# lorenzsp/EMRI_FrequencyDomainWaveforms

Hardware: AMD Instinct MI355X
Metric: FD waveforms/sec (2 yr, dt=10 s, ~3000 modes) at 1/2/4/8 GPUs; mode-sum HBM GB/s (higher is better)
Workload: dtype f64

## Files before the change

emri_frequencydomainwaveforms_amd/csrc/emrifd.hip:

```cpp

#include <hip/hip_runtime.h>

#include <cmath>
#include <cstdint>
#include <cstdlib>
#include <cstdio>
#include <algorithm>
#include <atomic>
#include <mutex>
#include <cstring>
#include <string>
#include <type_traits>

#include "../../include/emrifd.h"

#define EFD_VERSION 100

namespace {

constexpr int TILE = 256;
constexpr int NWAVE = TILE / 64;
#ifndef EFD_BPL
#define EFD_BPL 3
#endif
// ... 1141 lines not shown
        const int src = __ffsll((long long)sel) - 1;
        lg.m = __shfl(m, src, 64);
        lg.n = __shfl(n, src, 64);
        const int kg = __shfl(key, src, 64);
        const bool mine = lane < K && key == kg;
        if (mine) s_mem[eqb] = lane;
        lg.count = __popcll(__ballot(mine));
    }
    __syncthreads();
    return lg;
}
__global__ __launch_bounds__(64) void k_prep_pcr_b(const PrepBatch B) {
    PREP_WALKER(B);
    if (!(D.pcr & 1) || (int)blockIdx.x >= 4 + ((D.pcr & 2) ? 5 : 1) * D.K) return;
    const GroupAmpSrc ga{D.amp, D.ylm_p, D.ylm_m, D.sc_re, D.sc_im,
                         ws_at<int32_t>(W, L.gstart), ws_at<int32_t>(W, L.gmem)};
    __shared__ int s_mem[PCR_GROUPS_MAX_K];
    LocalGroups lg{};
    if (B.pcr_groups && (blockIdx.x == 0 || blockIdx.x >= 4))
        lg = pcr_local_groups(D, W, L, s_mem);
    prep_pcr_body(D.t, D.phi_phi, D.phi_r, D.f_phi, D.f_r, ga, lg, ws_at<int32_t>(W, L.gm),
                  ws_at<int32_t>(W, L.gn), D.nt, D.K,
                  ws_at<double>(W, L.coefT), ws_at<double>(W, L.kslope), ws_at<double>(W, L.coefA),
                  ws_at<int32_t>(W, L.runs), ws_at<Item>(W, L.items), ws_at<double>(W, L.invcp),
                  ws_at<double>(W, L.invdp), ws_at<Header>(W, L.header));
}

__global__ __launch_bounds__(64) void k_spline_shared(const double* __restrict__ x, int n,
                                                      const double* __restrict__ y, int ninterp,
                                                      double* coef, int64_t scratch_stride) {
    auto yf = [&](int i, int q) { return y[(size_t)i * ninterp + q]; };
    spline_shared(x, n, yf, ninterp, ninterp, coef, scratch_stride, blockIdx.x);
}

template <bool UPPER>
__device__ int64_t grid_bound(const double* __restrict__ f, int64_t nf, double v, int64_t g) {
    auto pred = [&](int64_t i) { return UPPER ? (f[i] > v) : (f[i] >= v); };
    g = g < 0 ? 0 : (g > nf ? nf : g);
    int64_t lo, hi;
    if (g < nf && !pred(g)) {
        lo = g + 1;
        int64_t step = 1;
        while (true) {
            const int64_t p = lo + step - 1;
            if (p >= nf) { hi = nf; break; }
            if (pred(p)) { hi = p; break; }
            lo = p + 1;
            step <<= 1;
        }
    } else {
        hi = g;
        int64_t step = 1;
        while (true) {
            const int64_t p = hi - step;
            if (p < 0) { lo = 0; break; }
            if (pred(p)) { hi = p; step <<= 1; }
            else { lo = p + 1; break; }
        }
    }
    while (lo < hi) {
        const int64_t mid = (lo + hi) >> 1;
        if (pred(mid)) hi = mid; else lo = mid + 1;
    }
    return lo;
}

__device__ bool build_item(
    const double* __restrict__ t, const double* __restrict__ f_phi, const double* __restrict__ f_r,
    const int32_t* __restrict__ gm, const int32_t* __restrict__ gn, int ni, int K,
    const double* __restrict__ coefA, const double* __restrict__ coefT,
    const int32_t* __restrict__ runs, const double* __restrict__ freq, int64_t nf, int paired,
    int64_t nl, int64_t nl1, Item* __restrict__ items, int4* __restrict__ ranges, int h, int j,
    unsigned long long& evals, bool env);

__device__ __forceinline__ void items_body(const double* __restrict__ t, const double* __restrict__ f_phi,
                        const double* __restrict__ f_r, const int32_t* __restrict__ gm,
                        const int32_t* __restrict__ gn, const int32_t* __restrict__ gstart,
                        int nt, int K, const double* __restrict__ coefA,
                        const double* __restrict__ coefT, const int32_t* __restrict__ runs,
                        const double* __restrict__ freq, int64_t nf, int paired, int64_t nl,
                        int64_t nl1, Item* __restrict__ items, int4* __restrict__ ranges,
                        Header* __restrict__ hdr, bool runs_mark, bool env) {
    const int ni = nt - 1;
    const int G = hdr->groups;
    const int64_t total = (int64_t)ni * G;
    if ((int64_t)blockIdx.x * blockDim.x >= total) return;
    const int64_t stride = (int64_t)gridDim.x * blockDim.x;
    __shared__ unsigned long long red[3][4];
    unsigned long long ev = 0, contrib = 0, eev = 0;
    for (int64_t gid = (int64_t)blockIdx.x * blockDim.x + threadIdx.x; gid < total;
         gid += stride) {
        const int g = (int)(gid % G), j = (int)(gid / G);
        if (runs_mark && j == 0 && runs[(size_t)g * 4 * MAXRUNS + 3] != 0)
            atomicOr(&hdr->runs_overflow, 1);
        unsigned long long e1 = 0;
        const bool envr = build_item(t, f_phi, f_r, gm, gn, ni, K, coefA, coefT, runs, freq, nf,
                                     paired, nl, nl1, items, ranges, g, j, e1, env);
        ev += e1;
        contrib += e1 * (unsigned long long)(gstart[g + 1] - gstart[g]);
        eev += envr ? e1 : 0;
    }
    for (int o = 32; o > 0; o >>= 1) {
        ev += __shfl_xor(ev, o);
        contrib += __shfl_xor(contrib, o);
        eev += __shfl_xor(eev, o);
    }
    if ((threadIdx.x & 63) == 0) {
        red[0][threadIdx.x >> 6] = contrib;
        red[1][threadIdx.x >> 6] = ev;
        red[2][threadIdx.x >> 6] = eev;
    }
    __syncthreads();
    if (threadIdx.x == 0) {
        const unsigned long long c = red[0][0] + red[0][1] + red[0][2] + red[0][3];
        const unsigned long long e = red[1][0] + red[1][1] + red[1][2] + red[1][3];
        const unsigned long long x = red[2][0] + red[2][1] + red[2][2] + red[2][3];
        if (c) atomicAdd((unsigned long long*)&hdr->contributions, c);
        if (e) atomicAdd((unsigned long long*)&hdr->evaluations, e);
        if (x) atomicAdd((unsigned long long*)&hdr->env_evaluations, x);
    }
}
__global__ __launch_bounds__(256) void k_items(const PrepBatch B) {
    PREP_WALKER(B);
    items_body(D.t, D.f_phi, D.f_r, ws_at<int32_t>(W, L.gm), ws_at<int32_t>(W, L.gn),
               ws_at<int32_t>(W, L.gstart), D.nt, D.K, ws_at<double>(W, L.coefA),
               ws_at<double>(W, L.coefT), ws_at<int32_t>(W, L.runs), D.freq, B.nf, B.paired, B.nl,
               B.nl1, ws_at<Item>(W, L.items), ws_at<int4>(W, L.ranges),
               ws_at<Header>(W, L.header), (D.pcr & 1) != 0, D.env != 0);
}

template <class FAT>
__device__ bool record_safe(const Item& it, FAT fat, int64_t lo0, int64_t hi0, int64_t lo1,
                            int64_t hi1) {
    double ga = INFINITY, gb = -INFINITY;
    if (hi0 > lo0) {
        const double fa = fat(0, lo0), fb = fat(1, hi0 - 1);
        ga = fmin(ga, fmin(-fa, -fb));
        gb = fmax(gb, fmax(-fa, -fb));
    }
    if (hi1 > lo1) {
        const double fa = fat(2, lo1), fb = fat(3, hi1 - 1);
        ga = fmin(ga, fmin(fa, fb));
        gb = fmax(gb, fmax(fa, fb));
    }
    if (!(ga <= gb)) return false;
    auto wat = [&](double g) {
        const double u = g - it.gx;
        const double tt = fma(fma(fma(it.ic[0], u, it.ic[1]), u, it.ic[2]), u, it.ic[3]);
        return tt - it.tj;
    };
    const double wa = wat(ga), wb = wat(gb);
    const double mg = 1e-6 * it.dtj;
    if (!(fmin(wa, wb) >= mg && fmax(wa, wb) <= it.dtj - mg)) return false;
    const double ua = ga - it.gx, ub = gb - it.gx;
    auto dt = [&](double u) { return fma(fma(3.0 * it.ic[0], u, 2.0 * it.ic[1]), u, it.ic[2]); };
    const double da = dt(ua), db = dt(ub);
    if (!((da > 0.0 && db > 0.0) || (da < 0.0 && db < 0.0))) return false;
    if (it.ic[0] != 0.0) {
        const double uv = -it.ic[1] / (3.0 * it.ic[0]);
        if (uv > ua && uv < ub) {
            const double dv = dt(uv);
            if (!((dv > 0.0) == (da > 0.0) && dv != 0.0)) return false;
        }
    }
    const double* f = it.fd;
    const double scale = fabs(f[0]) * it.dtj * it.dtj + fabs(f[1]) * it.dtj + fabs(f[2]);
    const double sg = (it.fdneg & 1) ? -1.0 : 1.0;
    auto fq = [&](double x) { return sg * fma(fma(f[0], x, f[1]), x, f[2]); };
    double fmn = fmin(fq(0.0), fq(it.dtj));
    if (f[0] != 0.0) {
        const double xv = -f[1] / (2.0 * f[0]);
        if (xv > 0.0 && xv < it.dtj) fmn = fmin(fmn, fq(xv));
    }
    return fmn > 1e-12 * scale && isfinite(scale);
}

__device__ bool build_item(
    const double* __restrict__ t, const double* __restrict__ f_phi, const double* __restrict__ f_r,
    const int32_t* __restrict__ gm, const int32_t* __restrict__ gn, int ni, int K,
    const double* __restrict__ coefA, const double* __restrict__ coefT,
    const int32_t* __restrict__ runs, const double* __restrict__ freq, int64_t nf, int paired,
    int64_t nl, int64_t nl1, Item* __restrict__ items, int4* __restrict__ ranges, int h, int j,
    unsigned long long& evals, bool env) {
    Item& it = items[(size_t)h * ni + j];
    const int m = gm[h], n = gn[h];
    const int32_t* rr = runs + (size_t)h * 4 * MAXRUNS;
    int run = -1;
    for (int r = 0; r < MAXRUNS; ++r) {
        if (rr[4 * r + 2] != 0 && j >= rr[4 * r] && j < rr[4 * r + 1]) { run = r; break; }
    }
    const int partner = (m != 0) ? 1 : 0;
    evals = 0;
    it.fdneg = 0;
    if (run < 0) {
        it.klo[0] = it.khi[0] = it.klo[1] = it.khi[1] = 0;
        ranges[(size_t)h * ni + j] = make_int4(0, 0, 0, 0);
        return false;
    }
    const int a = rr[4 * run], sg = rr[4 * run + 2];
    it.tj = t[j];
    it.dtj = t[j + 1] - t[j];
    const double dm = (double)m, dn = (double)n;
    for (int c = 0; c < 4; ++c) {
        const double* ca = coefA + ((size_t)j * 4 + c) * 4 * K + 4 * h;
        it.b[0][0][c] = ca[0];
        it.b[0][1][c] = ca[1];
        it.b[1][0][c] = ca[2];
        it.b[1][1][c] = ca[3];
        const double* ct = coefT + ((size_t)j * 4 + c) * 8;
        it.ph[c] = dm * ct[0] + dn * ct[1];
    }
    double gq[3], ymin_rec;
    {
        const double* ct = coefT + (size_t)j * 32;
        const double F0 = dm * ct[0 * 8 + 2] + dn * ct[0 * 8 + 3];
        const double F1 = dm * ct[1 * 8 + 2] + dn * ct[1 * 8 + 3];
        const double F2 = dm * ct[2 * 8 + 2] + dn * ct[2 * 8 + 3];
        it.fd[0] = 3.0 * F0; it.fd[1] = 2.0 * F1; it.fd[2] = F2;
        const double G0 = dm * ct[0 * 8 + 4] + dn * ct[0 * 8 + 5];
        const double G1 = dm * ct[1 * 8 + 4] + dn * ct[1 * 8 + 5];
        const double G2 = dm * ct[2 * 8 + 4] + dn * ct[2 * 8 + 5];
        it.fdd[0] = FDD_SCALE * (3.0 * G0);
        it.fdd[1] = FDD_SCALE * (2.0 * G1);
        it.fdd[2] = FDD_SCALE * G2;
        const double dt = it.dtj;
        auto qv = [](double a, double b, double c, double x) { return (a * x + b) * x + c; };
        const double fa = it.fd[2], fb = qv(it.fd[0], it.fd[1], it.fd[2], dt);
        it.fdneg = qv(it.fd[0], it.fd[1], it.fd[2], 0.5 * dt) < 0.0 ? 1 : 0;
        double fdmin = fmin(fabs(fa), fabs(fb));
        if ((fa > 0.0) != (fb > 0.0) || fa == 0.0 || fb == 0.0) fdmin = 0.0;
        if (it.fd[0] != 0.0) {
            const double xv = -it.fd[1] / (2.0 * it.fd[0]);
            if (xv > 0.0 && xv < dt) {
                const double fv = qv(it.fd[0], it.fd[1], it.fd[2], xv);
                if ((fv > 0.0) != (fa > 0.0)) fdmin = 0.0;
                fdmin = fmin(fdmin, fabs(fv));
            }
        }
        double gmax = fmax(fabs(G2), fabs(qv(3.0 * G0, 2.0 * G1, G2, dt)));
        if (G0 != 0.0) {
            const double xv = -(2.0 * G1) / (6.0 * G0);
            if (xv > 0.0 && xv < dt) gmax = fmax(gmax, fabs(qv(3.0 * G0, 2.0 * G1, G2, xv)));
        }
        const double ymin = gmax > 0.0 ? TWO_PI * fdmin * fdmin * fdmin / (3.0 * gmax * gmax) / 1.1
                                       : INFINITY;
        int J = FAST_J;
        for (int jj = 1; jj < FAST_J; ++jj)
            if (ymin >= JSER_Y[jj]) { J = jj; break; }
        it.jser = J;
        gq[0] = 3.0 * G0; gq[1] = 2.0 * G1; gq[2] = G2;
        ymin_rec = ymin;
    }
    const double Fj = knotF(f_phi, f_r, m, n, j), Fj1 = knotF(f_phi, f_r, m, n, j + 1);
    const double xlo = sg > 0 ? Fj : Fj1;
    const double xhi = sg > 0 ? Fj1 : Fj;
    const bool strict_lo = sg > 0 ? (j == a) : (j + 1 == rr[4 * run + 1]);
    const double f0 = freq[0], span = freq[nf - 1] - f0;
    const double gsc = span > 0.0 ? (double)(nf - 1) / span : 0.0;
    auto guess = [&](double v) { return (int64_t)floor((v - f0) * gsc); };
    const double bv[4] = {-xhi, -xlo, xlo, xhi};
    const bool bu[4] = {true, !strict_lo, strict_lo, false};
    int64_t bg[4];
    double b3[4][3];
#pragma unroll
    for (int q = 0; q < 4; ++q) {
        const int64_t g = guess(bv[q]);
        bg[q] = g < 0 ? 0 : (g > nf ? nf : g);
    }
#pragma unroll
    for (int q = 0; q < 4; ++q) {
        const int64_t g = bg[q];
        b3[q][0] = freq[g >= 1 ? g - 1 : 0];
        b3[q][1] = freq[g < nf ? g : nf - 1];
        b3[q][2] = freq[g + 1 < nf ? g + 1 : nf - 1];
    }
    int64_t bk[4];
#pragma unroll
    for (int q = 0; q < 4; ++q) {
        const double v = bv[q];
        const int64_t g = bg[q];
        auto pred = [&](double x) { return bu[q] ? (x > v) : (x >= v); };
        int64_t k = -1;
        if (!(g >= 1 && pred(b3[q][0]))) {
            if (g == nf) k = nf;
            else if (pred(b3[q][1])) k = g;
            else if (g + 1 == nf) k = nf;
            else if (pred(b3[q][2])) k = g + 1;
        }
        if (k < 0)
            k = bu[q] ? grid_bound<true>(freq, nf, v, g) : grid_bound<false>(freq, nf, v, g);
        bk[q] = k;
    }
    int64_t lo0 = bk[0], hi0 = bk[1], lo1 = bk[2], hi1 = bk[3];
    const int64_t lim0 = paired ? nl : nf;
    const int64_t lim1 = paired ? nl1 : (partner ? nf : 0);
    auto clampr = [](int64_t& lo, int64_t& hi, int64_t lim) {
        if (lo > lim) lo = lim;
        if (hi > lim) hi = lim;
        if (hi < lo) hi = lo;
    };
    clampr(lo0, hi0, lim0);
    clampr(lo1, hi1, lim1);
    it.klo[0] = (int32_t)lo0; it.khi[0] = (int32_t)hi0;
    it.klo[1] = (int32_t)lo1; it.khi[1] = (int32_t)hi1;
    ranges[(size_t)h * ni + j] = make_int4((int)lo0, (int)hi0, (int)lo1, (int)hi1);
    auto fat = [&](int q, int64_t x) {
        const int64_t g = bg[q];
        if (g >= 1 && x == g - 1) return b3[q][0];
        if (g < nf && x == g) return b3[q][1];
        if (g + 1 < nf && x == g + 1) return b3[q][2];
        return freq[x];
    };
    if (record_safe(it, fat, lo0, hi0, lo1, hi1)) it.fdneg |= 2;
    const int mult = paired ? 1 + partner : 1;
    evals = (unsigned long long)((hi0 - lo0) + (hi1 - lo1)) * mult;
    if (env && (it.fdneg & 2) && ymin_rec >= ENV_MIN_Y && evals > 0) {
        EnvFit E;
        if (env_fit(it.fd, gq, it.dtj, (it.fdneg & 1) != 0, E)) {
            double* e = env_of(&it);
            for (int c = 0; c <= ENV_DEG; ++c) e[c] = E.a[c] * ENV_AMP_SCALE;
            for (int c = 0; c < 4; ++c) it.ph[c] -= E.th[c];
            it.jser = 0;
            return true;
        }
    }
    return false;
}

__device__ __forceinline__ void slot_segment(int i, const int32_t* __restrict__ runs,
                                             const int4* __restrict__ ranges, int nt, int G,
                                             int lim0, int lim1, int2& lh, int4& info) {
    const int h = i / (2 * MAXRUNS), r = (i >> 1) % MAXRUNS, sb = i & 1;
    const int ni = nt - 1;
    lh = make_int2(0, 0);
    info = make_int4(0, 0, 0, 0);
    const int32_t* rr = runs + (size_t)h * 4 * MAXRUNS + 4 * r;
    if (h < G && rr[2] != 0) {
        const int ja = rr[0], jb = rr[1], n = jb - ja;
        const int dir = (sb == 0) ? -rr[2] : rr[2];
        const int lim = sb ? lim1 : lim0;
        const int4* rg = ranges + (size_t)h * ni;
        int lo = 0, hi = n;
        while (lo < hi) {
            const int mid = (lo + hi) >> 1;
            const int4 v = rg[dir > 0 ? ja + mid : jb - 1 - mid];
            if ((sb ? v.w : v.y) > 0) hi = mid; else lo = mid + 1;
        }
        const int pa = lo;
        hi = n;
        while (lo < hi) {
            const int mid = (lo + hi) >> 1;
            const int4 v = rg[dir > 0 ? ja + mid : jb - 1 - mid];
            if ((sb ? v.z : v.x) >= lim) hi = mid; else lo = mid + 1;
        }
        const int pb = lo;
        if (pb > pa) {
            const int4 rf = rg[dir > 0 ? ja + pa : jb - 1 - pa];
            const int4 rl = rg[dir > 0 ? ja + pb - 1 : jb - pb];
            const int klo = sb ? rf.z : rf.x, khi = sb ? rl.w : rl.y;
            if (khi > klo) {
                lh = make_int2(klo, khi);
                const int jfirst = dir > 0 ? ja + pa : jb - pb;
                info = make_int4(h * ni + jfirst, pb - pa, dir, sb);
            }
        }
    }
}
__device__ __forceinline__ void segment_slots_body(const int32_t* __restrict__ runs,
                                                       const int4* __restrict__ ranges, int nt,
                                                       int K, int lim0, int lim1,
                                                       const Header* __restrict__ hdr,
                                                       int2* __restrict__ slot_lh,
                                                       int4* __restrict__ slot_info,
                                                       int32_t* __restrict__ blockcnt,
                                                       int32_t* __restrict__ blocktiles) {
    const int i = blockIdx.x * blockDim.x + threadIdx.x;
    __shared__ int wc[4], wt[4];
    int ntl = 0;
    bool valid = false;
    if (i < K * MAXRUNS * 2) {
        const int G = hdr->groups;
        int2 lh;
        int4 info;
        slot_segment(i, runs, ranges, nt, G, lim0, lim1, lh, info);
        slot_lh[i] = lh;
        slot_info[i] = info;
        valid = info.y > 0;
        if (valid) ntl = (lh.y - 1) / TILE_LANES - lh.x / TILE_LANES + 1;
    }
    const unsigned long long bal = __ballot(valid);
    int tsum = ntl;
    for (int o = 32; o > 0; o >>= 1) tsum += __shfl_xor(tsum, o);
    if ((threadIdx.x & 63) == 0) {
        wc[threadIdx.x >> 6] = __popcll(bal);
        wt[threadIdx.x >> 6] = tsum;
    }
    __syncthreads();
    if (threadIdx.x == 0) {
        blockcnt[blockIdx.x] = wc[0] + wc[1] + wc[2] + wc[3];
        blocktiles[blockIdx.x] = wt[0] + wt[1] + wt[2] + wt[3];
    }
}
__device__ __forceinline__ int slot_blocks(int K) { return (2 * MAXRUNS * K + 255) / 256; }
__global__ __launch_bounds__(256) void k_segment_slots(const PrepBatch B) {
    PREP_WALKER(B);
    if ((int)blockIdx.x >= slot_blocks(D.K)) return;
    segment_slots_body(ws_at<int32_t>(W, L.runs), ws_at<int4>(W, L.ranges), D.nt, D.K,
                       (int)(B.paired ? B.nl : B.nf), (int)(B.paired ? B.nl1 : B.nf),
                       ws_at<Header>(W, L.header), ws_at<int2>(W, L.slotlh),
// ... 1542 lines not shown
    const int32_t w_lo = (int32_t)(tile * TILE_LANES + wave * 64 * BPL);
    double llacc = 0.0;
#pragma unroll
    for (int i = 0; i < BPL; ++i) {
        const int64_t k = w_lo + 64 * i + lane;
        if (k >= nlanes) continue;
        const int64_t km = nf - 1 - k;
        double2 sk = make_double2(0.0, 0.0);
        double2 sm = make_double2(0.0, 0.0);
        if (km == k) {
            sk.x += sm.x;
            sk.y += sm.y;
            sm = sk;
        }
        auto put = [&](int64_t j, double2 a, double2 b) {
            if (j < k0) return;
            double2 vp = make_double2(0.5 * (a.x + b.x), 0.5 * (a.y - b.y));
            double2 vc = make_double2(-0.5 * (a.y + b.y), 0.5 * (a.x - b.x));
            {
#pragma clang fp contract(off)
                const int64_t q = j - k0, nb = nf - k0;
                const double2 d0 = reinterpret_cast<const double2*>(lld)[q];
                const double2 d1 = reinterpret_cast<const double2*>(lld)[nb + q];
                const double w0 = llw[q], w1 = llw[nb + q];
                const double r0 = d0.x - vp.x * w0, i0 = d0.y - vp.y * w0;
                const double r1 = d1.x - vc.x * w1, i1 = d1.y - vc.y * w1;
                llacc = fma(r0, r0, fma(i0, i0, llacc));
                llacc = fma(r1, r1, fma(i1, i1, llacc));
            }
        };
        put(km, sm, sk);
        if (km != k) put(k, sk, sm);
    }
#pragma unroll
    for (int o = 32; o > 0; o >>= 1) llacc += __shfl_xor(llacc, o, 64);
    __shared__ double llw4[NWAVE];
    if (lane == 0) llw4[wave] = llacc;
    __syncthreads();
    if (tid == 0) {
        double t = 0.0;
#pragma unroll
        for (int w = 0; w < NWAVE; ++w) t += llw4[w];
        llconst[tile] = t;
    }
}

struct LlBatch {
    const double* part[EFD_BATCH_MAX];
    const Header* hdr[EFD_BATCH_MAX];
    double* out;
    const double* llconst;
    int64_t ntiles;
    int32_t n;
};
struct StatusBatch {
    Header* h[EFD_BATCH_MAX];
    int32_t n;
};
__global__ __launch_bounds__(64) void k_lane_gather(const StatusBatch sb, int32_t* out) {
    const int i = threadIdx.x;
    if (i >= sb.n) return;
    out[2 * i] = sb.h[i]->lane_lo;
    out[2 * i + 1] = sb.h[i]->lane_hi;
}
__global__ __launch_bounds__(64) void k_status_gather(const StatusBatch sb, int32_t* out) {
    const int i = threadIdx.x;
    if (i >= sb.n) return;
    Header* h = sb.h[i];
    const int32_t f = (h->runs_overflow ? 1 : 0) | (h->bad_mn ? 2 : 0) | (h->bad_tile ? 4 : 0);
    out[i] = f;
    if (f) {
        h->runs_overflow = 0;
        h->bad_mn = 0;
        h->bad_tile = 0;
    }
}

__global__ __launch_bounds__(256) void k_ll_final(const LlBatch lb) {
    ll_final_reduce(lb.part[blockIdx.x], lb.hdr[blockIdx.x], lb.llconst, lb.ntiles,
                           lb.out + blockIdx.x);
}

constexpr int TK_HITS = TILE;
constexpr int TK_ROWS = 8;
__device__ __forceinline__ void tile_keys_body(
    const int4* __restrict__ ranges, const int2* __restrict__ seglh,
    const int4* __restrict__ seginfo, const int32_t* __restrict__ nsegp,
    const int32_t* __restrict__ segbase, const int32_t* __restrict__ stb0,
    const int32_t* __restrict__ stb1, int64_t ntiles, uint32_t* __restrict__ tkeys,
    int32_t* __restrict__ tcnt) {
    static_assert(SEGWIN == TILE, "one segment per thread and window row");
    __shared__ int hits[TK_HITS], hp0[TK_HITS], hcnt[TK_HITS], hoff[TK_HITS], hws[TK_HITS],
        hwt[TK_HITS];
    __shared__ int4 hinfo[TK_HITS];
    __shared__ int wcnt[TK_ROWS * NWAVE];
    __shared__ int part[NWAVE];
    const int64_t tile = blockIdx.x;
    if (tile >= ntiles) return;
    const int tid = threadIdx.x, lane = tid & 63;
    const int wave = __builtin_amdgcn_readfirstlane(tid >> 6);
    const int32_t tlo = (int32_t)(tile * TILE_LANES), thi = tlo + TILE_LANES;
    const int nseg = *nsegp;
#ifdef EFD_EXP
    if (tile == 0 && tid == 0) atomicAdd(&g_exp_count[27], (unsigned long long)nseg);
#endif
    int nhit = 0;
    for (int base = 0; base < nseg; base += TK_ROWS * TILE) {
        unsigned long long bal[TK_ROWS];
#pragma unroll
        for (int r = 0; r < TK_ROWS; ++r) {
            const int sgi = base + r * TILE + tid;
            bool hit = false;
            if (sgi < nseg) {
                const int2 lh = seglh[sgi];
                hit = lh.y > tlo && lh.x < thi;
            }
            bal[r] = __ballot(hit);
            if (lane == 0) wcnt[r * NWAVE + wave] = __popcll(bal[r]);
        }
        __syncthreads();
#pragma unroll
        for (int r = 0; r < TK_ROWS; ++r) {
            int before = nhit;
            for (int w = 0; w < wave; ++w) before += wcnt[r * NWAVE + w];
            if ((bal[r] >> lane) & 1ull) {
                const int pos = before + __popcll(bal[r] & ((1ull << lane) - 1ull));
                if (pos < TK_HITS) hits[pos] = base + r * TILE + tid;
            }
#pragma unroll
            for (int w = 0; w < NWAVE; ++w) nhit += wcnt[r * NWAVE + w];
        }
        __syncthreads();
    }
#ifdef EFD_EXP
    if (tid == 0) atomicAdd(&g_exp_count[28], (unsigned long long)nhit);
#endif
    if (nhit > TK_HITS) {
        if (tid == 0) tcnt[tile] = -1;
        return;
    }
    int c = 0;
    if (tid < nhit) {
        const int sg = hits[tid];
        const int32_t sbase = segbase[sg];
        const int4 info = seginfo[sg];
        int p0 = 0;
        if (sbase != SEG_NO_STB) {
            p0 = stb0[sbase + tile];
            c = max(stb1[sbase + tile] - p0, 0);
        } else {
            const int base = info.x, n = info.y, dir = info.z, sb = info.w;
            int lo = 0, hi = n;
            while (lo < hi) {
                const int mid = (lo + hi) >> 1;
                const int4 rg = ranges[base + (dir > 0 ? mid : n - 1 - mid)];
                if ((sb ? rg.w : rg.y) > tlo) hi = mid; else lo = mid + 1;
            }
            p0 = lo;
            hi = n;
            while (lo < hi) {
                const int mid = (lo + hi) >> 1;
                const int4 rg = ranges[base + (dir > 0 ? mid : n - 1 - mid)];
                if ((sb ? rg.z : rg.x) >= thi) hi = mid; else lo = mid + 1;
            }
            c = lo - p0;
        }
        hp0[tid] = p0;
        hcnt[tid] = c;
        hinfo[tid] = info;
    }
    int incl = c;
#pragma unroll
    for (int o = 1; o < 64; o <<= 1) {
        const int v = __shfl_up(incl, o, 64);
        if (lane >= o) incl += v;
    }
    if (lane == 63) part[wave] = incl;
    __syncthreads();
    int total = 0, woff = 0;
#pragma unroll
    for (int w = 0; w < NWAVE; ++w) {
        woff += w < wave ? part[w] : 0;
        total += part[w];
    }
    if (total > KEYCAP) {
        if (tid == 0) tcnt[tile] = -1;
        return;
    }
    if (tid < nhit) hoff[tid] = woff + incl - c;
    __syncthreads();
    {
        const int w = tid < nhit ? hits[tid] / SEGWIN : INT32_MAX;
        const bool first = tid < nhit && (tid == 0 || hits[tid - 1] / SEGWIN != w);
        const bool last = tid < nhit && (tid == nhit - 1 || hits[tid + 1] / SEGWIN != w);
        int st = first ? woff + incl - c : INT32_MIN;
        int en = last ? woff + incl : INT32_MAX;
#pragma unroll
        for (int o = 1; o < 64; o <<= 1) {
            const int vs = __shfl_up(st, o, 64), ve = __shfl_down(en, o, 64);
            if (lane >= o) st = max(st, vs);
            if (lane + o < 64) en = min(en, ve);
        }
        if (lane == 63) hws[wave] = st;
        if (lane == 0) hwt[wave] = en;
        __syncthreads();
        for (int v = 0; v < wave; ++v) st = max(st, hws[v]);
        for (int v = NWAVE - 1; v > wave; --v) en = min(en, hwt[v]);
        __syncthreads();
        if (tid < nhit) {
            hws[tid] = st;
            hwt[tid] = en - st;
        }
    }
    __syncthreads();
    uint32_t* out = tkeys + (size_t)tile * KEYCAP;
    for (int g = tid; g < total; g += TILE) {
        int lo = 0, hi = nhit - 1;
        while (lo < hi) {
            const int mid = (lo + hi + 1) >> 1;
            if (hoff[mid] <= g) lo = mid; else hi = mid - 1;
        }
        const int4 info = hinfo[lo];
        const int p = hp0[lo] + (g - hoff[lo]);
        const int j = info.z > 0 ? p : info.y - 1 - p;
        const int ws = hws[lo], take = hwt[lo];
        const int P = (take % 97) ? 97 : 101;
        out[ws + (int)(((unsigned)(g - ws) * (unsigned)P) % (unsigned)take)] =
            ((uint32_t)(info.x + j) << 1) | (uint32_t)info.w;
    }
    if (tid == 0) tcnt[tile] = total;
}
__global__ __launch_bounds__(TILE) void k_tile_keys(const PrepBatch B) {
    PREP_WALKER(B);
    if (D.lists == 0) return;
    tile_keys_body(ws_at<int4>(W, L.ranges), ws_at<int2>(W, L.seglh), ws_at<int4>(W, L.seginfo),
                   ws_at<int32_t>(W, L.nseg), ws_at<int32_t>(W, L.segbase),
                   ws_at<int32_t>(W, L.stb0), ws_at<int32_t>(W, L.stb1), L.ntiles,
                   ws_at<uint32_t>(W, L.tkeys), ws_at<int32_t>(W, L.tcnt));
}
#undef EFD_MODESUM_PARAMS
#undef EFD_MODESUM_ARGS

constexpr int ORDER_BUCKETS = 64;
__device__ __forceinline__ int tile_cost_bucket(int32_t c) {
    if (c < 0) return ORDER_BUCKETS - 1;
    const float l = __log2f((float)c + 1.0f) * 4.0f;
    return min((int)l, ORDER_BUCKETS - 2);
}
__device__ __forceinline__ int wave_bucket_add(int* hist, int bucket, bool valid) {
    const int lane = threadIdx.x & 63;
    unsigned long long todo = __ballot(valid);
    int res = 0;
    while (todo) {
        const int leader = __ffsll((long long)todo) - 1;
        const int bl = __shfl(bucket, leader, 64);
        const unsigned long long same = __ballot(valid && bucket == bl) & todo;
        int base = 0;
        if (lane == leader) base = atomicAdd(&hist[bl], __popcll(same));
        base = __shfl(base, leader, 64);
        if ((same >> lane) & 1ull) res = base + __popcll(same & ((1ull << lane) - 1ull));
        todo &= ~same;
    }
    return res;
}
__device__ __forceinline__ void tile_order_body(const int32_t* __restrict__ tcnt,
                                                int64_t ntiles, int32_t* __restrict__ tperm) {
    __shared__ int hist[ORDER_BUCKETS];
    const int tid = threadIdx.x;
    if (tid < ORDER_BUCKETS) hist[tid] = 0;
    __syncthreads();
    constexpr int PER = 16;
    int bk[PER];
#pragma unroll
    for (int q = 0; q < PER; ++q) {
        const int64_t i = tid + (int64_t)q * 1024;
        bk[q] = i < ntiles ? tile_cost_bucket(tcnt[i]) : -1;
    }
#pragma unroll
    for (int q = 0; q < PER; ++q) wave_bucket_add(hist, bk[q], bk[q] >= 0);
    const int64_t npass = (ntiles + 1023) / 1024;
    for (int64_t p = PER; p < npass; ++p) {
        const int64_t i = tid + p * 1024;
        const int bkt = i < ntiles ? tile_cost_bucket(tcnt[i]) : 0;
        wave_bucket_add(hist, bkt, i < ntiles);
    }
    __syncthreads();
    if (tid == 0) {
        int acc = 0;
        for (int q = ORDER_BUCKETS - 1; q >= 0; --q) { const int h = hist[q]; hist[q] = acc; acc += h; }
    }
    __syncthreads();
#pragma unroll
    for (int q = 0; q < PER; ++q) {
        const int pos = wave_bucket_add(hist, bk[q], bk[q] >= 0);
        if (bk[q] >= 0) tperm[pos] = (int32_t)(tid + q * 1024);
    }
    for (int64_t p = PER; p < npass; ++p) {
        const int64_t i = tid + p * 1024;
        const int bkt = i < ntiles ? tile_cost_bucket(tcnt[i]) : 0;
        const int pos = wave_bucket_add(hist, bkt, i < ntiles);
        if (i < ntiles) tperm[pos] = (int32_t)i;
    }
}
__global__ __launch_bounds__(1024) void k_tile_order(const PrepBatch B) {
    PREP_WALKER(B);
    if (D.lists != 3) return;
    tile_order_body(ws_at<int32_t>(W, L.tcnt), L.ntiles, ws_at<int32_t>(W, L.tperm));
}

constexpr int TD_THREADS = 256;
constexpr int TD_SPL = 4;

__device__ __forceinline__ int knot_interval(const double* __restrict__ t, int nt, double x) {
// ... 1257 lines not shown
        any_order |= d.lists == 3;
#ifdef EFD_EXP_NO_PCR
        const bool pcr = false;
#else
        const bool pcr = ai->nt >= 4 && ai->nt <= PCR_NMAX;
#endif
        d.pcr = pcr ? (ai->K < PCR_MAX_K ? 3 : 1) : 0;
        if (pcr) {
            any_pcr = true;
            ntmax_pcr = std::max(ntmax_pcr, ai->nt);
            pcr_blocks = std::max(pcr_blocks, 4 + (d.pcr == 3 ? 5 : 1) * ai->K);
        }
        if (d.pcr != 3) any_thomas = true;
        ntmax = std::max(ntmax, ai->nt);
        Kmax = std::max(Kmax, ai->K);
        nimax = std::max(nimax, ai->nt - 1);
        const int64_t per = ai->K >= ITEMS_SPLIT_K ? ITEMS_PER_THREAD_K : 1;
        items_max = std::max(items_max, ((int64_t)(ai->nt - 1) * ai->K + per - 1) / per);
        if (i == 0) {
            B.paired = paired;
            B.nf = ai->nf;
            B.nl = L.nlanes;
            B.nl1 = paired ? ((ai->nf % 2) ? L.nlanes - 1 : L.nlanes) : ai->nf;
            ntiles = L.ntiles;
        }
    }
    (void)nimax;
    hipStream_t st = (hipStream_t)stream;
    const unsigned nz = (unsigned)count;
    B.pcr_groups = (!any_thomas && Kmax <= PCR_GROUPS_MAX_K) ? 1 : 0;
    {
        if (!B.pcr_groups) {
            hipLaunchKernelGGL(k_group_b, dim3(1, 1, nz), dim3(256), 0, st, B);
            HIP_TRY(hipGetLastError());
        }
        if (any_thomas) {
            const int gper = Kmax >= ITEMS_SPLIT_K ? ITEMS_PER_THREAD_K : 1;
            hipLaunchKernelGGL(k_group_amp_b, dim3((Kmax / gper + 255) / 256, ntmax, nz),
                               dim3(256), 0, st, B);
            HIP_TRY(hipGetLastError());
        }
    }
    {
        if (any_pcr) {
            hipLaunchKernelGGL(k_prep_pcr_b, dim3(pcr_blocks, 1, nz), dim3(64),
                               sizeof(double) * 9 * ntmax_pcr, st, B);
            HIP_TRY(hipGetLastError());
        }
        if (any_thomas) {
            const int nb = 1 + (4 * Kmax + 63) / 64 + (Kmax + 63) / 64;
            hipLaunchKernelGGL(k_prep_b, dim3(nb, 1, nz), dim3(64), sizeof(double) * 7 * ntmax,
                               st, B);
            HIP_TRY(hipGetLastError());
        }
    }
    {
        const int64_t blocks = (items_max + 255) / 256;
        hipLaunchKernelGGL(k_items, dim3((unsigned)blocks, 1, nz), dim3(256), 0, st, B);
        HIP_TRY(hipGetLastError());
    }
    if (Kmax <= SEG1_MAX_K) {
        int64_t need = 0;
        for (int i = 0; i < count; ++i) {
            const int64_t b = (int64_t)a[i]->K * (a[i]->nt - 1) * 16;
            if (b <= SEG1_LDS_CAP) need = std::max(need, b);
        }
        B.seg_lds = (int32_t)need;
        B.split_min = split_min_cost();
        hipLaunchKernelGGL(k_segments_one, dim3(1, 1, nz), dim3(SEG1_NT), (size_t)B.seg_lds, st,
                           B);
        HIP_TRY(hipGetLastError());
    } else {
        const int nslot = Kmax * MAXRUNS * 2;
        const int nblk = (nslot + 255) / 256;
        hipLaunchKernelGGL(k_segment_slots, dim3(nblk, 1, nz), dim3(256), 0, st, B);
        HIP_TRY(hipGetLastError());
        hipLaunchKernelGGL(k_segment_compact, dim3(nblk, 1, nz), dim3(256), 0, st, B);
        HIP_TRY(hipGetLastError());
        hipLaunchKernelGGL(k_seg_tiles, dim3((unsigned)std::min(nslot, 1024), 1, nz), dim3(256),
                           0, st, B);
        HIP_TRY(hipGetLastError());
    }
    if (any_lists) {
        hipLaunchKernelGGL(k_tile_keys, dim3((unsigned)ntiles, 1, nz), dim3(TILE), 0, st, B);
        HIP_TRY(hipGetLastError());
    }
    if (any_order) {
        hipLaunchKernelGGL(k_tile_order, dim3(1, 1, nz), dim3(1024), 0, st, B);
        HIP_TRY(hipGetLastError());
    }
    return EFD_OK;
}

static int modesum_impl(const efd_modesum_args* a, void* workspace, size_t workspace_bytes,
                        void* stream, int phase) {
    {
        const int rc = check_modesum_args(a, workspace, phase);
        if (rc != EFD_OK) return rc;
    }
    const int paired = a->grid_symmetric ? 1 : 0;
    const Layout L = make_layout(a->nt, a->K, a->nf, paired);
    if (workspace_bytes < L.total)
        return fail(EFD_ERR_WORKSPACE, "efd_modesum: workspace too small (see efd_modesum_workspace_bytes)");

    hipStream_t st = (hipStream_t)stream;
    char* ws = (char*)workspace;
    Header* hdr = (Header*)(ws + L.header);
    const Item* items = (const Item*)(ws + L.items);
    const int4* ranges = (const int4*)(ws + L.ranges);
    const int2* seglh = (const int2*)(ws + L.seglh);
    const int4* seginfo = (const int4*)(ws + L.seginfo);
    const int32_t* nseg = (const int32_t*)(ws + L.nseg);
    const int32_t* gm = (const int32_t*)(ws + L.gm);
    const int32_t* gn = (const int32_t*)(ws + L.gn);
    const double* coefA = (const double*)(ws + L.coefA);
    const double* coefT = (const double*)(ws + L.coefT);
    const double2* sctab_g = (const double2*)(ws + L.sctab);
    const uint32_t* tkeys = (const uint32_t*)(ws + L.tkeys);
    int32_t* tcnt = (int32_t*)(ws + L.tcnt);
    const int32_t* segbase = (const int32_t*)(ws + L.segbase);
    const int32_t* stb0 = (const int32_t*)(ws + L.stb0);
    const int32_t* stb1 = (const int32_t*)(ws + L.stb1);
    const int nt = a->nt, K = a->K;
    const int64_t nf = a->nf;
    const int64_t nl = L.nlanes;

    if (phase & 1) {
        const int rc = prepare_batch_impl("efd_modesum_prepare", &a, &workspace, &workspace_bytes,
                                          1, stream);
        if (rc != EFD_OK) return rc;
    }
    if (phase & 2) {
        const int64_t gq = 8 * XCD_GROUP;
        const dim3 grid((unsigned)((L.ntiles + gq - 1) / gq * gq)), block(TILE);
        const int acc = a->accumulate ? 1 : 0;
        if (a->prof_begin) HIP_TRY(hipEventRecord((hipEvent_t)a->prof_begin, st));
        int32_t* tcnt_sum = use_prebuilt(K) ? tcnt : nullptr;
        const int32_t* tperm =
            use_cost_order(L, K)
                ? (const int32_t*)(ws + L.tperm) : nullptr;
#define EFD_LAUNCH(P, C)                                                                      \
    hipLaunchKernelGGL((k_modesum<P, C, BPL>), grid, block, 0, st, items, ranges, seglh,          \
                       seginfo, nseg, a->freq, nf, nl, L.ntiles, nt, K, gm, gn, a->t, coefA,      \
                       coefT, sctab_g, tkeys, tcnt_sum, tperm, segbase, stb0, stb1, hdr, acc,      \
                       a->out, a->hp, a->hc, a->k0)
        if (paired) {
            if (a->caustic == EFD_CAUSTIC_UNIFORM) EFD_LAUNCH(true, EFD_CAUSTIC_UNIFORM);
            else EFD_LAUNCH(true, EFD_CAUSTIC_SPA);
        } else {
            if (a->caustic == EFD_CAUSTIC_UNIFORM) EFD_LAUNCH(false, EFD_CAUSTIC_UNIFORM);
            else EFD_LAUNCH(false, EFD_CAUSTIC_SPA);
        }
#undef EFD_LAUNCH
        HIP_TRY(hipGetLastError());
        if (a->prof_end) HIP_TRY(hipEventRecord((hipEvent_t)a->prof_end, st));
    }
    return EFD_OK;
}

int efd_modesum(const efd_modesum_args* a, void* workspace, size_t workspace_bytes, void* stream) {
    return modesum_impl(a, workspace, workspace_bytes, stream, 3);
}

int efd_modesum_prepare(const efd_modesum_args* a, void* workspace, size_t workspace_bytes,
                        void* stream) {
    return modesum_impl(a, workspace, workspace_bytes, stream, 1);
}
// ... 657 lines not shown
```

Before: 1923.

## Restructure tile-key builder to one wave per tile and vectorize item record writes

The tile-key kernel now gives each tile a single wavefront instead of a whole block. Block-wide syncs and cross-wave scans become wave-local ballots, shuffles and wave barriers, and hit metadata is packed into fewer LDS arrays. build_item preloads its inputs, writes the Item record with 16-byte vector stores in place of scattered scalar stores, and k_items replaces its shuffle reduction with LDS atomics plus a waves-per-EU hint. The risks are contention on the LDS atomics, the hard-coded struct offset assumptions, and a limit of 12 bits on window fields.

```diff
diff --git a/emri_frequencydomainwaveforms_amd/csrc/emrifd.hip b/emri_frequencydomainwaveforms_amd/csrc/emrifd.hip
--- a/emri_frequencydomainwaveforms_amd/csrc/emrifd.hip
+++ b/emri_frequencydomainwaveforms_amd/csrc/emrifd.hip
@@ -1247,12 +1247,13 @@
                         int64_t nl1, Item* __restrict__ items, int4* __restrict__ ranges,
                         Header* __restrict__ hdr, bool runs_mark, bool env) {
     const int ni = nt - 1;
-    const int G = hdr->groups;
+    const int G = __builtin_amdgcn_readfirstlane(hdr->groups);
     const int64_t total = (int64_t)ni * G;
     if ((int64_t)blockIdx.x * blockDim.x >= total) return;
     const int64_t stride = (int64_t)gridDim.x * blockDim.x;
-    __shared__ unsigned long long red[3][4];
-    unsigned long long ev = 0, contrib = 0, eev = 0;
+    __shared__ unsigned long long red[3];
+    if (threadIdx.x < 3) red[threadIdx.x] = 0;
+    __syncthreads();
     for (int64_t gid = (int64_t)blockIdx.x * blockDim.x + threadIdx.x; gid < total;
          gid += stride) {
         const int g = (int)(gid % G), j = (int)(gid / G);
@@ -1261,31 +1262,22 @@
         unsigned long long e1 = 0;
         const bool envr = build_item(t, f_phi, f_r, gm, gn, ni, K, coefA, coefT, runs, freq, nf,
                                      paired, nl, nl1, items, ranges, g, j, e1, env);
-        ev += e1;
-        contrib += e1 * (unsigned long long)(gstart[g + 1] - gstart[g]);
-        eev += envr ? e1 : 0;
-    }
-    for (int o = 32; o > 0; o >>= 1) {
-        ev += __shfl_xor(ev, o);
-        contrib += __shfl_xor(contrib, o);
-        eev += __shfl_xor(eev, o);
-    }
-    if ((threadIdx.x & 63) == 0) {
-        red[0][threadIdx.x >> 6] = contrib;
-        red[1][threadIdx.x >> 6] = ev;
-        red[2][threadIdx.x >> 6] = eev;
+        if (e1) {
+            atomicAdd(&red[0], e1 * (unsigned long long)(gstart[g + 1] - gstart[g]));
+            atomicAdd(&red[1], e1);
+            if (envr) atomicAdd(&red[2], e1);
+        }
     }
     __syncthreads();
     if (threadIdx.x == 0) {
-        const unsigned long long c = red[0][0] + red[0][1] + red[0][2] + red[0][3];
-        const unsigned long long e = red[1][0] + red[1][1] + red[1][2] + red[1][3];
-        const unsigned long long x = red[2][0] + red[2][1] + red[2][2] + red[2][3];
+        const unsigned long long c = red[0], e = red[1], x = red[2];
         if (c) atomicAdd((unsigned long long*)&hdr->contributions, c);
         if (e) atomicAdd((unsigned long long*)&hdr->evaluations, e);
         if (x) atomicAdd((unsigned long long*)&hdr->env_evaluations, x);
     }
 }
-__global__ __launch_bounds__(256) void k_items(const PrepBatch B) {
+__global__ __launch_bounds__(256) __attribute__((amdgpu_waves_per_eu(4))) void k_items(
+    const PrepBatch B) {
     PREP_WALKER(B);
     items_body(D.t, D.f_phi, D.f_r, ws_at<int32_t>(W, L.gm), ws_at<int32_t>(W, L.gn),
                ws_at<int32_t>(W, L.gstart), D.nt, D.K, ws_at<double>(W, L.coefA),
@@ -1347,47 +1339,68 @@
     const int32_t* __restrict__ runs, const double* __restrict__ freq, int64_t nf, int paired,
     int64_t nl, int64_t nl1, Item* __restrict__ items, int4* __restrict__ ranges, int h, int j,
     unsigned long long& evals, bool env) {
-    Item& it = items[(size_t)h * ni + j];
+    Item& out = items[(size_t)h * ni + j];
     const int m = gm[h], n = gn[h];
     const int32_t* rr = runs + (size_t)h * 4 * MAXRUNS;
-    int run = -1;
+    int3 rv[MAXRUNS];
+#pragma unroll
+    for (int r = 0; r < MAXRUNS; ++r) rv[r] = make_int3(rr[4 * r], rr[4 * r + 1], rr[4 * r + 2]);
+    const double tj0 = t[j], tj1 = t[j + 1];
+    const double fp0 = f_phi[j], fp1 = f_phi[j + 1], fr0 = f_r[j], fr1 = f_r[j + 1];
+    const double f0 = freq[0], fend = freq[nf - 1];
+    double cT[4][6];
+#pragma unroll
+    for (int c = 0; c < 4; ++c)
+#pragma unroll
+        for (int q = 0; q < 6; ++q) cT[c][q] = coefT[((size_t)j * 4 + c) * 8 + q];
+    Item it;
+    int a = 0, jb = 0, sg = 0;
+#pragma unroll
     for (int r = 0; r < MAXRUNS; ++r) {
-        if (rr[4 * r + 2] != 0 && j >= rr[4 * r] && j < rr[4 * r + 1]) { run = r; break; }
+        if (sg == 0 && rv[r].z != 0 && j >= rv[r].x && j < rv[r].y) {
+            a = rv[r].x; jb = rv[r].y; sg = rv[r].z;
+        }
     }
     const int partner = (m != 0) ? 1 : 0;
     evals = 0;
     it.fdneg = 0;
-    if (run < 0) {
-        it.klo[0] = it.khi[0] = it.klo[1] = it.khi[1] = 0;
+    if (sg == 0) {
+        out.fdneg = 0;
+        *reinterpret_cast<int4*>(&out.klo[0]) = make_int4(0, 0, 0, 0);
         ranges[(size_t)h * ni + j] = make_int4(0, 0, 0, 0);
         return false;
     }
-    const int a = rr[4 * run], sg = rr[4 * run + 2];
-    it.tj = t[j];
-    it.dtj = t[j + 1] - t[j];
+    it.tj = tj0;
+    out.tj = tj0;
+    it.dtj = tj1 - tj0;
     const double dm = (double)m, dn = (double)n;
-    for (int c = 0; c < 4; ++c) {
-        const double* ca = coefA + ((size_t)j * 4 + c) * 4 * K + 4 * h;
-        it.b[0][0][c] = ca[0];
-        it.b[0][1][c] = ca[1];
-        it.b[1][0][c] = ca[2];
-        it.b[1][1][c] = ca[3];
-        const double* ct = coefT + ((size_t)j * 4 + c) * 8;
-        it.ph[c] = dm * ct[0] + dn * ct[1];
-    }
+    {
+        double2 cA[4][2];
+#pragma unroll
+        for (int c = 0; c < 4; ++c) {
+            const double2* ca =
+                reinterpret_cast<const double2*>(coefA + ((size_t)j * 4 + c) * 4 * K + 4 * h);
+            cA[c][0] = ca[0];
+            cA[c][1] = ca[1];
+        }
+        double2* bp = reinterpret_cast<double2*>(&out.b[0][0][0]);
+        bp[0] = make_double2(cA[0][0].x, cA[1][0].x); bp[1] = make_double2(cA[2][0].x, cA[3][0].x);
+        bp[2] = make_double2(cA[0][0].y, cA[1][0].y); bp[3] = make_double2(cA[2][0].y, cA[3][0].y);
+        bp[4] = make_double2(cA[0][1].x, cA[1][1].x); bp[5] = make_double2(cA[2][1].x, cA[3][1].x);
+        bp[6] = make_double2(cA[0][1].y, cA[1][1].y); bp[7] = make_double2(cA[2][1].y, cA[3][1].y);
+    }
+    double2* const p = reinterpret_cast<double2*>(&out.ph[0]);
+    p[0] = make_double2(dm * cT[0][0] + dn * cT[0][1], dm * cT[1][0] + dn * cT[1][1]);
+    p[1] = make_double2(dm * cT[2][0] + dn * cT[2][1], dm * cT[3][0] + dn * cT[3][1]);
     double gq[3], ymin_rec;
     {
-        const double* ct = coefT + (size_t)j * 32;
-        const double F0 = dm * ct[0 * 8 + 2] + dn * ct[0 * 8 + 3];
-        const double F1 = dm * ct[1 * 8 + 2] + dn * ct[1 * 8 + 3];
-        const double F2 = dm * ct[2 * 8 + 2] + dn * ct[2 * 8 + 3];
+        const double F0 = dm * cT[0][2] + dn * cT[0][3];
+        const double F1 = dm * cT[1][2] + dn * cT[1][3];
+        const double F2 = dm * cT[2][2] + dn * cT[2][3];
         it.fd[0] = 3.0 * F0; it.fd[1] = 2.0 * F1; it.fd[2] = F2;
-        const double G0 = dm * ct[0 * 8 + 4] + dn * ct[0 * 8 + 5];
-        const double G1 = dm * ct[1 * 8 + 4] + dn * ct[1 * 8 + 5];
-        const double G2 = dm * ct[2 * 8 + 4] + dn * ct[2 * 8 + 5];
-        it.fdd[0] = FDD_SCALE * (3.0 * G0);
-        it.fdd[1] = FDD_SCALE * (2.0 * G1);
-        it.fdd[2] = FDD_SCALE * G2;
+        const double G0 = dm * cT[0][4] + dn * cT[0][5];
+        const double G1 = dm * cT[1][4] + dn * cT[1][5];
+        const double G2 = dm * cT[2][4] + dn * cT[2][5];
         const double dt = it.dtj;
         auto qv = [](double a, double b, double c, double x) { return (a * x + b) * x + c; };
         const double fa = it.fd[2], fb = qv(it.fd[0], it.fd[1], it.fd[2], dt);
@@ -1416,11 +1429,12 @@
         gq[0] = 3.0 * G0; gq[1] = 2.0 * G1; gq[2] = G2;
         ymin_rec = ymin;
     }
-    const double Fj = knotF(f_phi, f_r, m, n, j), Fj1 = knotF(f_phi, f_r, m, n, j + 1);
+    const double Fj = __dadd_rn(__dmul_rn(dm, fp0), __dmul_rn(dn, fr0));
+    const double Fj1 = __dadd_rn(__dmul_rn(dm, fp1), __dmul_rn(dn, fr1));
     const double xlo = sg > 0 ? Fj : Fj1;
     const double xhi = sg > 0 ? Fj1 : Fj;
-    const bool strict_lo = sg > 0 ? (j == a) : (j + 1 == rr[4 * run + 1]);
-    const double f0 = freq[0], span = freq[nf - 1] - f0;
+    const bool strict_lo = sg > 0 ? (j == a) : (j + 1 == jb);
+    const double span = fend - f0;
     const double gsc = span > 0.0 ? (double)(nf - 1) / span : 0.0;
     auto guess = [&](double v) { return (int64_t)floor((v - f0) * gsc); };
     const double bv[4] = {-xhi, -xlo, xlo, xhi};
@@ -1466,8 +1480,7 @@
     };
     clampr(lo0, hi0, lim0);
     clampr(lo1, hi1, lim1);
-    it.klo[0] = (int32_t)lo0; it.khi[0] = (int32_t)hi0;
-    it.klo[1] = (int32_t)lo1; it.khi[1] = (int32_t)hi1;
+    *reinterpret_cast<int4*>(&out.klo[0]) = make_int4((int)lo0, (int)lo1, (int)hi0, (int)hi1);
     ranges[(size_t)h * ni + j] = make_int4((int)lo0, (int)hi0, (int)lo1, (int)hi1);
     auto fat = [&](int q, int64_t x) {
         const int64_t g = bg[q];
@@ -1476,20 +1489,38 @@
         if (g + 1 < nf && x == g + 1) return b3[q][2];
         return freq[x];
     };
+    it.gx = out.gx;
+#pragma unroll
+    for (int c = 0; c < 4; ++c) it.ic[c] = out.ic[c];
     if (record_safe(it, fat, lo0, hi0, lo1, hi1)) it.fdneg |= 2;
     const int mult = paired ? 1 + partner : 1;
     evals = (unsigned long long)((hi0 - lo0) + (hi1 - lo1)) * mult;
+    static_assert(ENV_DEG + 1 == 7, "fd[3], dtj, fdd[3]: the envelope's slots");
+    double w[ENV_DEG + 1] = {it.fd[0], it.fd[1], it.fd[2], it.dtj,
+                             FDD_SCALE * gq[0], FDD_SCALE * gq[1], FDD_SCALE * gq[2]};
+    bool envr = false;
     if (env && (it.fdneg & 2) && ymin_rec >= ENV_MIN_Y && evals > 0) {
         EnvFit E;
         if (env_fit(it.fd, gq, it.dtj, (it.fdneg & 1) != 0, E)) {
-            double* e = env_of(&it);
-            for (int c = 0; c <= ENV_DEG; ++c) e[c] = E.a[c] * ENV_AMP_SCALE;
-            for (int c = 0; c < 4; ++c) it.ph[c] -= E.th[c];
+#pragma unroll
+            for (int c = 0; c <= ENV_DEG; ++c) w[c] = E.a[c] * ENV_AMP_SCALE;
+            asm volatile("" ::: "memory");
+            const double2 q0 = p[0], q1 = p[1];
+            p[0] = make_double2(q0.x - E.th[0], q0.y - E.th[1]);
+            p[1] = make_double2(q1.x - E.th[2], q1.y - E.th[3]);
             it.jser = 0;
-            return true;
-        }
-    }
-    return false;
+            envr = true;
+        }
+    }
+    static_assert(offsetof(Item, ph) % 16 == 0 && offsetof(Item, fd) == offsetof(Item, ph) + 32 &&
+                  offsetof(Item, jser) == offsetof(Item, ph) + 88 &&
+                  offsetof(Item, fdneg) == offsetof(Item, jser) + 4, "the record's 16-B pieces");
+    p[2] = make_double2(w[0], w[1]);
+    p[3] = make_double2(w[2], w[3]);
+    p[4] = make_double2(w[4], w[5]);
+    reinterpret_cast<int4*>(p)[5] =
+        make_int4(__double2loint(w[6]), __double2hiint(w[6]), it.jser, it.fdneg);
+    return envr;
 }
 
 __device__ __forceinline__ void slot_segment(int i, const int32_t* __restrict__ runs,
@@ -3198,153 +3229,168 @@
 }
 
 constexpr int TK_HITS = TILE;
-constexpr int TK_ROWS = 8;
+constexpr int TK_ROUNDS = 8;
+constexpr int TK_HROUNDS = TK_HITS / 64;
+__device__ __forceinline__ void wave_lds_sync() {
+    __builtin_amdgcn_fence(__ATOMIC_RELEASE, "wavefront");
+    __builtin_amdgcn_wave_barrier();
+    __builtin_amdgcn_fence(__ATOMIC_ACQUIRE, "wavefront");
+}
 __device__ __forceinline__ void tile_keys_body(
     const int4* __restrict__ ranges, const int2* __restrict__ seglh,
     const int4* __restrict__ seginfo, const int32_t* __restrict__ nsegp,
     const int32_t* __restrict__ segbase, const int32_t* __restrict__ stb0,
     const int32_t* __restrict__ stb1, int64_t ntiles, uint32_t* __restrict__ tkeys,
     int32_t* __restrict__ tcnt) {
-    static_assert(SEGWIN == TILE, "one segment per thread and window row");
-    __shared__ int hits[TK_HITS], hp0[TK_HITS], hcnt[TK_HITS], hoff[TK_HITS], hws[TK_HITS],
-        hwt[TK_HITS];
-    __shared__ int4 hinfo[TK_HITS];
-    __shared__ int wcnt[TK_ROWS * NWAVE];
-    __shared__ int part[NWAVE];
-    const int64_t tile = blockIdx.x;
+    __shared__ int s_hits[NWAVE][TK_HITS], s_hoff[NWAVE][TK_HITS], s_hrec[NWAVE][TK_HITS],
+        s_hwin[NWAVE][TK_HITS];
+    constexpr int HW_BITS = 12, HW_MASK = (1 << HW_BITS) - 1;
+    constexpr int HW_DIR = 2 * HW_BITS, HW_SB = 2 * HW_BITS + 1;
+    static_assert(KEYCAP <= HW_MASK, "a window's start and key count fit HW_BITS each");
+    const int lane = threadIdx.x & 63;
+    const int wave = __builtin_amdgcn_readfirstlane(threadIdx.x >> 6);
+    const int64_t tile = (int64_t)blockIdx.x * NWAVE + wave;
     if (tile >= ntiles) return;
-    const int tid = threadIdx.x, lane = tid & 63;
-    const int wave = __builtin_amdgcn_readfirstlane(tid >> 6);
+    int* const hits = s_hits[wave];
+    int* const hoff = s_hoff[wave];
+    int* const hrec = s_hrec[wave];
+    int* const hwin = s_hwin[wave];
     const int32_t tlo = (int32_t)(tile * TILE_LANES), thi = tlo + TILE_LANES;
     const int nseg = *nsegp;
 #ifdef EFD_EXP
-    if (tile == 0 && tid == 0) atomicAdd(&g_exp_count[27], (unsigned long long)nseg);
+    if (tile == 0 && lane == 0) atomicAdd(&g_exp_count[27], (unsigned long long)nseg);
 #endif
     int nhit = 0;
-    for (int base = 0; base < nseg; base += TK_ROWS * TILE) {
-        unsigned long long bal[TK_ROWS];
-#pragma unroll
-        for (int r = 0; r < TK_ROWS; ++r) {
-            const int sgi = base + r * TILE + tid;
-            bool hit = false;
-            if (sgi < nseg) {
-                const int2 lh = seglh[sgi];
-                hit = lh.y > tlo && lh.x < thi;
+    for (int base = 0; base < nseg; base += TK_ROUNDS * 64) {
+        int2 lh[TK_ROUNDS];
+#pragma unroll
+        for (int r = 0; r < TK_ROUNDS; ++r) {
+            const int sgi = base + r * 64 + lane;
+            lh[r] = sgi < nseg ? seglh[sgi] : make_int2(INT32_MAX, INT32_MIN);
+        }
+#pragma unroll
+        for (int r = 0; r < TK_ROUNDS; ++r) {
+            const bool hit = lh[r].y > tlo && lh[r].x < thi;
+            const unsigned long long bal = __ballot(hit);
+            if (hit) {
+                const int pos = nhit + __popcll(bal & ((1ull << lane) - 1ull));
+                if (pos < TK_HITS) hits[pos] = base + r * 64 + lane;
             }
-            bal[r] = __ballot(hit);
-            if (lane == 0) wcnt[r * NWAVE + wave] = __popcll(bal[r]);
-        }
-        __syncthreads();
-#pragma unroll
-        for (int r = 0; r < TK_ROWS; ++r) {
-            int before = nhit;
-            for (int w = 0; w < wave; ++w) before += wcnt[r * NWAVE + w];
-            if ((bal[r] >> lane) & 1ull) {
-                const int pos = before + __popcll(bal[r] & ((1ull << lane) - 1ull));
-                if (pos < TK_HITS) hits[pos] = base + r * TILE + tid;
-            }
-#pragma unroll
-            for (int w = 0; w < NWAVE; ++w) nhit += wcnt[r * NWAVE + w];
-        }
-        __syncthreads();
+            nhit += __popcll(bal);
+        }
     }
 #ifdef EFD_EXP
-    if (tid == 0) atomicAdd(&g_exp_count[28], (unsigned long long)nhit);
+    if (lane == 0) atomicAdd(&g_exp_count[28], (unsigned long long)nhit);
 #endif
     if (nhit > TK_HITS) {
-        if (tid == 0) tcnt[tile] = -1;
+        if (lane == 0) tcnt[tile] = -1;
         return;
     }
-    int c = 0;
-    if (tid < nhit) {
-        const int sg = hits[tid];
-        const int32_t sbase = segbase[sg];
-        const int4 info = seginfo[sg];
-        int p0 = 0;
-        if (sbase != SEG_NO_STB) {
-            p0 = stb0[sbase + tile];
-            c = max(stb1[sbase + tile] - p0, 0);
-        } else {
-            const int base = info.x, n = info.y, dir = info.z, sb = info.w;
-            int lo = 0, hi = n;
-            while (lo < hi) {
-                const int mid = (lo + hi) >> 1;
-                const int4 rg = ranges[base + (dir > 0 ? mid : n - 1 - mid)];
-                if ((sb ? rg.w : rg.y) > tlo) hi = mid; else lo = mid + 1;
-            }
-            p0 = lo;
-            hi = n;
-            while (lo < hi) {
-                const int mid = (lo + hi) >> 1;
-                const int4 rg = ranges[base + (dir > 0 ? mid : n - 1 - mid)];
-                if ((sb ? rg.z : rg.x) >= thi) hi = mid; else lo = mid + 1;
-            }
-            c = lo - p0;
-        }
-        hp0[tid] = p0;
-        hcnt[tid] = c;
-        hinfo[tid] = info;
-    }
-    int incl = c;
-#pragma unroll
-    for (int o = 1; o < 64; o <<= 1) {
-        const int v = __shfl_up(incl, o, 64);
-        if (lane >= o) incl += v;
-    }
-    if (lane == 63) part[wave] = incl;
-    __syncthreads();
-    int total = 0, woff = 0;
-#pragma unroll
-    for (int w = 0; w < NWAVE; ++w) {
-        woff += w < wave ? part[w] : 0;
-        total += part[w];
+    wave_lds_sync();
+    int sg[TK_HROUNDS], sbase[TK_HROUNDS], p0[TK_HROUNDS], c[TK_HROUNDS];
+    int4 info[TK_HROUNDS];
+#pragma unroll
+    for (int r = 0; r < TK_HROUNDS; ++r) {
+        const int i = r * 64 + lane;
+        sg[r] = i < nhit ? hits[i] : 0;
+        sbase[r] = SEG_NO_STB;
+        info[r] = make_int4(0, 0, 1, 0);
+        if (i < nhit) {
+            sbase[r] = segbase[sg[r]];
+            info[r] = seginfo[sg[r]];
+        }
+    }
+#pragma unroll
+    for (int r = 0; r < TK_HROUNDS; ++r) {
+        p0[r] = c[r] = 0;
+        if (sbase[r] != SEG_NO_STB) {
+            p0[r] = stb0[sbase[r] + tile];
+            c[r] = max(stb1[sbase[r] + tile] - p0[r], 0);
+        }
+    }
+#pragma unroll
+    for (int r = 0; r < TK_HROUNDS; ++r) {
+        if (sbase[r] != SEG_NO_STB) continue;
+        const int base = info[r].x, n = info[r].y, dir = info[r].z, sb = info[r].w;
+        int lo = 0, hi = n;
+        while (lo < hi) {
+            const int mid = (lo + hi) >> 1;
+            const int4 rg = ranges[base + (dir > 0 ? mid : n - 1 - mid)];
+            if ((sb ? rg.w : rg.y) > tlo) hi = mid; else lo = mid + 1;
+        }
+        p0[r] = lo;
+        hi = n;
+        while (lo < hi) {
+            const int mid = (lo + hi) >> 1;
+            const int4 rg = ranges[base + (dir > 0 ? mid : n - 1 - mid)];
+            if ((sb ? rg.z : rg.x) >= thi) hi = mid; else lo = mid + 1;
+        }
+        c[r] = lo - p0[r];
+    }
+    int off[TK_HROUNDS], total = 0;
+#pragma unroll
+    for (int r = 0; r < TK_HROUNDS; ++r) {
+        int incl = c[r];
+#pragma unroll
+        for (int o = 1; o < 64; o <<= 1) {
+            const int v = __shfl_up(incl, o, 64);
+            if (lane >= o) incl += v;
+        }
+        off[r] = total + incl - c[r];
+        total += __shfl(incl, 63, 64);
     }
     if (total > KEYCAP) {
-        if (tid == 0) tcnt[tile] = -1;
+        if (lane == 0) tcnt[tile] = -1;
         return;
     }
-    if (tid < nhit) hoff[tid] = woff + incl - c;
-    __syncthreads();
-    {
-        const int w = tid < nhit ? hits[tid] / SEGWIN : INT32_MAX;
-        const bool first = tid < nhit && (tid == 0 || hits[tid - 1] / SEGWIN != w);
-        const bool last = tid < nhit && (tid == nhit - 1 || hits[tid + 1] / SEGWIN != w);
-        int st = first ? woff + incl - c : INT32_MIN;
-        int en = last ? woff + incl : INT32_MAX;
+    int st[TK_HROUNDS], en[TK_HROUNDS];
+#pragma unroll
+    for (int r = 0; r < TK_HROUNDS; ++r) {
+        const int i = r * 64 + lane;
+        const bool in = i < nhit;
+        const int w = sg[r] / SEGWIN;
+        const bool first = in && (i == 0 || hits[i - 1] / SEGWIN != w);
+        const bool last = in && (i == nhit - 1 || hits[i + 1] / SEGWIN != w);
+        st[r] = first ? off[r] : INT32_MIN;
+        en[r] = last ? off[r] + c[r] : INT32_MAX;
 #pragma unroll
         for (int o = 1; o < 64; o <<= 1) {
-            const int vs = __shfl_up(st, o, 64), ve = __shfl_down(en, o, 64);
-            if (lane >= o) st = max(st, vs);
-            if (lane + o < 64) en = min(en, ve);
-        }
-        if (lane == 63) hws[wave] = st;
-        if (lane == 0) hwt[wave] = en;
-        __syncthreads();
-        for (int v = 0; v < wave; ++v) st = max(st, hws[v]);
-        for (int v = NWAVE - 1; v > wave; --v) en = min(en, hwt[v]);
-        __syncthreads();
-        if (tid < nhit) {
-            hws[tid] = st;
-            hwt[tid] = en - st;
-        }
-    }
-    __syncthreads();
+            const int vs = __shfl_up(st[r], o, 64), ve = __shfl_down(en[r], o, 64);
+            if (lane >= o) st[r] = max(st[r], vs);
+            if (lane + o < 64) en[r] = min(en[r], ve);
+        }
+    }
+#pragma unroll
+    for (int r = 1; r < TK_HROUNDS; ++r) st[r] = max(st[r], __shfl(st[r - 1], 63, 64));
+#pragma unroll
+    for (int r = TK_HROUNDS - 2; r >= 0; --r) en[r] = min(en[r], __shfl(en[r + 1], 0, 64));
+#pragma unroll
+    for (int r = 0; r < TK_HROUNDS; ++r) {
+        const int i = r * 64 + lane;
+        if (i < nhit) {
+            const bool fwd = info[r].z > 0;
+            hoff[i] = off[r];
+            hrec[i] = fwd ? info[r].x + p0[r] - off[r] : info[r].x + info[r].y - 1 - p0[r] + off[r];
+            hwin[i] = st[r] | ((en[r] - st[r]) << HW_BITS) | ((fwd ? 1 : 0) << HW_DIR) |
+                      (info[r].w << HW_SB);
+        }
+    }
+    wave_lds_sync();
     uint32_t* out = tkeys + (size_t)tile * KEYCAP;
-    for (int g = tid; g < total; g += TILE) {
+    for (int g = lane; g < total; g += 64) {
         int lo = 0, hi = nhit - 1;
         while (lo < hi) {
             const int mid = (lo + hi + 1) >> 1;
             if (hoff[mid] <= g) lo = mid; else hi = mid - 1;
         }
-        const int4 info = hinfo[lo];
-        const int p = hp0[lo] + (g - hoff[lo]);
-        const int j = info.z > 0 ? p : info.y - 1 - p;
-        const int ws = hws[lo], take = hwt[lo];
+        const int hw = hwin[lo];
+        const int rec = ((hw >> HW_DIR) & 1) ? hrec[lo] + g : hrec[lo] - g;
+        const int ws = hw & HW_MASK, take = (hw >> HW_BITS) & HW_MASK;
         const int P = (take % 97) ? 97 : 101;
         out[ws + (int)(((unsigned)(g - ws) * (unsigned)P) % (unsigned)take)] =
-            ((uint32_t)(info.x + j) << 1) | (uint32_t)info.w;
-    }
-    if (tid == 0) tcnt[tile] = total;
+            ((uint32_t)rec << 1) | (uint32_t)((hw >> HW_SB) & 1);
+    }
+    if (lane == 0) tcnt[tile] = total;
 }
 __global__ __launch_bounds__(TILE) void k_tile_keys(const PrepBatch B) {
     PREP_WALKER(B);
@@ -4768,7 +4814,8 @@
         HIP_TRY(hipGetLastError());
     }
     if (any_lists) {
-        hipLaunchKernelGGL(k_tile_keys, dim3((unsigned)ntiles, 1, nz), dim3(TILE), 0, st, B);
+        hipLaunchKernelGGL(k_tile_keys, dim3((unsigned)((ntiles + NWAVE - 1) / NWAVE), 1, nz),
+                           dim3(TILE), 0, st, B);
         HIP_TRY(hipGetLastError());
     }
     if (any_order) {
```

Result: no change. 1940 (median of 6 runs) (+0.9%).
